# broadinstitute/delphy

Hardware: AMD Instinct MI355X
Metric: MCMC moves/sec on 100k-tip SARS-CoV-2 EMAT at 1/2/4/8 MI355X (higher is better)
Workload: dtype f64; 1 GPU; C4: synthetic 100000-tip EMAT, 29903 sites, HKY(kappa=5) + skygrid, 8092 partition parts (199999 nodes), 1000 moves/part/step, move mix 7.5/7.5/15/1/1; parts_per_gpu=8092, parts_requested=8192, max_part_nodes=-1, lds_staging=True, tickets_per_part_and_pass=4, parallelism=parts sharded over 1 GPU(s), one wavefront per part, collectives=none (one rank), emat_build_id=7d9b3896ecee7423

## Files before the change

### delphy_amd/csrc/emat_debug_host.hpp

```cpp
#ifndef EMAT_DEBUG_HOST_HPP_
#define EMAT_DEBUG_HOST_HPP_

namespace {

emat_status debug_settle(emat_backend* h, bool need_derived) {
  emat_status st = emat_synchronize(h); if (st) return st;
  st = sync_model_to_device(h); if (st) return st;
  st = materialize(h); if (st) return st;
  return need_derived && !h->derived_valid ? launch_recalc(h) : EMAT_OK;
}

}

extern "C" {

emat_status emat_debug_slab_layout(emat_backend* h, int32_t part_id, uint32_t* out8) {
  if (!h || !out8 || part_id < 0 || part_id >= (int)h->parts.size()) return EMAT_ERR_INVALID_ARGUMENT;
  if (!h->have_coal) return fail(h, EMAT_ERR_STATE, "no coalescent parts built");
  const PartHost& ph = h->parts[part_id];
  const int trace_cap = h->cfg.trace_moves > 0 ? h->cfg.trace_moves : 0;
  const uint32_t content = heap_content_bytes(ph.tree);
  const SlabGeo g = slab_geometry(h, ph.tree.num_nodes(), ph.tree.num_muts(), content, (int)ph.coal.k_bar_p.size(), ph.includes_run_root, ph.space_boost, ph.cell_boost);
  out8[0] = (uint32_t)sizeof(SlabHeader); out8[1] = (uint32_t)ph.tree.num_nodes() * (uint32_t)sizeof(NodeRec) + miss_dl_bytes_for((uint32_t)ph.tree.num_nodes()); out8[2] = a16((uint32_t)g.cell_cap * cell_bytes_for(ph.includes_run_root));
  out8[3] = a16((uint32_t)trace_cap * 32u); out8[4] = content; out8[5] = g.heap; out8[6] = g.scratch; out8[7] = (uint32_t)g.cell_cap;
  return EMAT_OK;
}
emat_status emat_debug_gamma(emat_backend* h, int32_t mode, int32_t n, const double* a, const double* x_or_q, double* out) {
  if (!h || n < 0 || (mode != 0 && mode != 1) || (n > 0 && (!a || !x_or_q || !out))) return EMAT_ERR_INVALID_ARGUMENT;
  if (h->host_only) return no_device(h);
  if (!bind_device(h)) return fail(h, EMAT_ERR_HIP, "hipSetDevice failed");
  if (n == 0) return EMAT_OK;
  DevBuf<double> da, dx, dout;
  HIP_TRY(da.upload(a, (size_t)n)); HIP_TRY(dx.upload(x_or_q, (size_t)n)); HIP_TRY(dout.upload(x_or_q, (size_t)n));
  hipLaunchKernelGGL(k_debug_gamma, dim3((unsigned)((n + 63) / 64)), dim3(64), 0, h->stream, da.p, dx.p, dout.p, n, mode);
  HIP_TRY(hipGetLastError());
  HIP_TRY(hipStreamSynchronize(h->stream));
  HIP_TRY(hipMemcpy(out, dout.p, (size_t)n * sizeof(double), hipMemcpyDeviceToHost));
  return EMAT_OK;
}
emat_status emat_debug_pop(emat_backend* h, const emat_pop_model* pm, int32_t op, int32_t n, const double* a, const double* b, double* out) {
  if (!h || !pm || n < 0 || op < 0 || op > 2 || (n > 0 && (!a || !b || !out))) return EMAT_ERR_INVALID_ARGUMENT;
  if (h->host_only) return no_device(h);
  if (!bind_device(h)) return fail(h, EMAT_ERR_HIP, "hipSetDevice failed");
  if (n == 0) return EMAT_OK;
  HostPopModel hp;
  try { hp = HostPopModel::from_c(*pm); } catch (const std::exception& ex) { return fail(h, EMAT_ERR_INVALID_ARGUMENT, ex.what()); }
  DevBuf<double> dx, dg, da, db, dout;
  HIP_TRY(dx.upload(hp.x.data(), hp.x.size())); HIP_TRY(dg.upload(hp.gamma.data(), hp.gamma.size()));
  HIP_TRY(da.upload(a, (size_t)n)); HIP_TRY(db.upload(b, (size_t)n)); HIP_TRY(dout.alloc((size_t)n));
  PopTable pt{};
  pt.kind = hp.kind; pt.skygrid_type = hp.skygrid_type; pt.skygrid_num_knots = (int)hp.x.size();
  for (int i = 0; i < 4; ++i) pt.p[i] = hp.p[i];
  pt.t_c = hp.t_c; pt.skygrid_x = dx.p; pt.skygrid_gamma = dg.p;
  pt.skygrid_inv_dx = (hp.x.size() >= 2 && hp.x.back() > hp.x.front()) ? (double)(hp.x.size() - 1) / (hp.x.back() - hp.x.front()) : 0.0;
  hipLaunchKernelGGL(k_debug_pop, dim3((unsigned)((n + 63) / 64)), dim3(64), 0, h->stream, pt, (int)op, da.p, db.p, dout.p, (int)n);
  HIP_TRY(hipGetLastError());
  HIP_TRY(hipStreamSynchronize(h->stream));
  HIP_TRY(hipMemcpy(out, dout.p, (size_t)n * sizeof(double), hipMemcpyDeviceToHost));
  return EMAT_OK;
}
emat_status emat_debug_interval_op(emat_backend* h, int32_t op, const int32_t* a, int32_t na, const int32_t* b, int32_t nb, int32_t* out, int32_t* n_out) {
  if (!h || !n_out || na < 0 || nb < 0 || (na > 0 && !a) || (nb > 0 && !b) || !out) return EMAT_ERR_INVALID_ARGUMENT;
  if (h->host_only) return no_device(h);
  if (!bind_device(h)) return fail(h, EMAT_ERR_HIP, "hipSetDevice failed");
  DevBuf<IvRec> dA, dB, dO; DevBuf<int> dn;
  HIP_TRY(dA.upload((const IvRec*)a, (size_t)na)); HIP_TRY(dB.upload((const IvRec*)b, (size_t)(op == 5 ? 0 : nb))); HIP_TRY(dO.alloc((size_t)(na + nb + 1))); HIP_TRY(dn.alloc(1));
  hipLaunchKernelGGL(k_debug_interval_op, dim3(1), dim3(64), 0, h->stream, (int)op, dA.p, (int)na, dB.p, (int)(op == 5 ? 0 : nb), op == 5 && nb > 0 ? b[0] : 0, dO.p, dn.p);
  HIP_TRY(hipGetLastError());
  HIP_TRY(hipStreamSynchronize(h->stream));
  int cnt = 0;
  HIP_TRY(hipMemcpy(&cnt, dn.p, sizeof(int), hipMemcpyDeviceToHost));
  if (cnt < 0) return fail(h, EMAT_ERR_INVALID_ARGUMENT, "emat_debug_interval_op: unknown op");
  *n_out = cnt;
  if (op <= 3 && cnt > 0) HIP_TRY(hipMemcpy(out, dO.p, (size_t)cnt * sizeof(IvRec), hipMemcpyDeviceToHost));
  return EMAT_OK;
}
emat_status emat_debug_tree_query(emat_backend* h, int32_t part_id, int32_t op, int32_t n, const int32_t* a, const int32_t* b, int32_t* out) {
  if (!h || n < 0 || (op != 0 && op != 1) || (n > 0 && (!a || !b || !out))) return EMAT_ERR_INVALID_ARGUMENT;
  if (h->host_only) return no_device(h);
  if (!bind_device(h)) return fail(h, EMAT_ERR_HIP, "hipSetDevice failed");
  if (part_id < 0 || part_id >= (int)h->parts.size()) return EMAT_ERR_INVALID_ARGUMENT;
  const int nn = h->parts[part_id].n_nodes;
  for (int i = 0; i < n; ++i) if (a[i] < -1 || a[i] >= nn || b[i] < -1 || b[i] >= nn) return fail(h, EMAT_ERR_INVALID_ARGUMENT, "emat_debug_tree_query: node index out of range");
  if (n == 0) return EMAT_OK;
  emat_status st = debug_settle(h, false); if (st) return st;
  DevBuf<int32_t> da, db, dout;
  HIP_TRY(da.upload(a, (size_t)n)); HIP_TRY(db.upload(b, (size_t)n)); HIP_TRY(dout.alloc((size_t)n));
  KernelArgs ka = make_args(h);
  hipLaunchKernelGGL(k_debug_tree_query, dim3(1), dim3(k_wave), 0, h->stream, ka, (int)part_id, (int)op, da.p, db.p, dout.p, (int)n);
  HIP_TRY(hipGetLastError());
  HIP_TRY(hipStreamSynchronize(h->stream));
  HIP_TRY(hipMemcpy(out, dout.p, (size_t)n * sizeof(int32_t), hipMemcpyDeviceToHost));
  return EMAT_OK;
}
emat_status emat_debug_miss_dl_check(emat_backend* h, int32_t* out_2n) {
  if (!h || !out_2n) return EMAT_ERR_INVALID_ARGUMENT;
  if (h->host_only) return no_device(h);
  if (!bind_device(h)) return fail(h, EMAT_ERR_HIP, "hipSetDevice failed");
  if (h->parts.empty()) return EMAT_OK;
  emat_status st = debug_settle(h, false); if (st) return st;
  DevBuf<int32_t> dout;
  HIP_TRY(dout.alloc(2 * h->parts.size()));
  return run_over_parts(h, k_debug_miss_dl_check, dout.p, out_2n, 2 * h->parts.size(), dout.p);
}
emat_status emat_debug_graft(emat_backend* h, int32_t part_id, int32_t X, double mu_proposal, int32_t mode, int32_t new_sibling, double new_t_P,
                             double* out, int32_t out_cap, int32_t* out_len) {
  if (!h || !out || !out_len || out_cap < 2 || mode < 0 || mode > 3) return EMAT_ERR_INVALID_ARGUMENT;
  if (h->host_only) return no_device(h);
  if (!bind_device(h)) return fail(h, EMAT_ERR_HIP, "hipSetDevice failed");
  if (part_id < 0 || part_id >= (int)h->parts.size()) return EMAT_ERR_INVALID_ARGUMENT;
  const int nn = h->parts[part_id].n_nodes;
  if (X < 0 || X >= nn || (mode == 3 && (new_sibling < 0 || new_sibling >= nn))) return fail(h, EMAT_ERR_INVALID_ARGUMENT, "emat_debug_graft: node index out of range");
  emat_status st = debug_settle(h, true); if (st) return st;
  DevBuf<double> dout; DevBuf<int32_t> dlen;
  HIP_TRY(dout.alloc((size_t)out_cap)); HIP_TRY(dlen.alloc(1));
  KernelArgs ka = make_args(h);
  hipLaunchKernelGGL(k_debug_graft, dim3(1), dim3(k_wave), 0, h->stream, ka, (int)part_id, (int)X, mu_proposal, (int)mode, (int)new_sibling, new_t_P, dout.p, (int)out_cap, dlen.p);
  HIP_TRY(hipGetLastError());
  HIP_TRY(hipStreamSynchronize(h->stream));
  HIP_TRY(hipMemcpy(out_len, dlen.p, sizeof(int32_t), hipMemcpyDeviceToHost));
  HIP_TRY(hipMemcpy(out, dout.p, (size_t)std::min(*out_len, out_cap) * sizeof(double), hipMemcpyDeviceToHost));
  if (mode >= 1) h->device_wrote_slabs();
  if (out[0] != 0.0) return fail(h, EMAT_ERR_INTERNAL, "emat_debug_graft: the device code stopped with part status " + std::to_string((int)out[0]));
  return *out_len > out_cap ? fail(h, EMAT_ERR_CAPACITY, "emat_debug_graft: out_cap too small") : EMAT_OK;
}
emat_status emat_debug_sample_history(emat_backend* h, int32_t part_id, int32_t n, const int32_t* branch, const double* t_end, const uint8_t* start_seq, double T, double mu,
                                      int32_t* counts, double* muts, int32_t muts_cap, int32_t* num_muts) {
// ... 134 lines not shown
```

### delphy_amd/csrc/emat_device_core.hpp

```cpp
#ifndef EMAT_DEV_NS
#error "define EMAT_DEV_NS and EMAT_VARIANT_LDS before including the device headers"
#endif

#include <hip/hip_runtime.h>
#include <cfloat>
#include <cstdint>

#include "emat_slab.hpp"

#ifndef EMAT_DEVICE_COMMON_ONCE_
#define EMAT_DEVICE_COMMON_ONCE_
namespace emat {
extern __shared__ __attribute__((aligned(16))) uint8_t emat_lds[];
constexpr uint32_t k_lds_tables_bytes = k_max_lds_partitions * (1 + 4 + 16) * 8;
constexpr uint32_t k_lds_ctx_bytes = 288;
#ifndef EMAT_RNG_BLOCKS
#define EMAT_RNG_BLOCKS 32
#endif
constexpr uint32_t k_rng_blocks = EMAT_RNG_BLOCKS;
static_assert(k_rng_blocks == 0 || (k_rng_blocks <= 64 && (k_rng_blocks & (k_rng_blocks - 1)) == 0), "one block per lane, a power of two");
constexpr uint32_t k_lds_rng_bytes = k_rng_blocks * 16;
constexpr uint32_t k_lds_static_bytes = k_lds_tables_bytes + k_lds_ctx_bytes + k_lds_rng_bytes + k_max_lds_partitions * 16 * 8;
__shared__ __attribute__((aligned(16))) uint8_t emat_lds_tables[k_lds_tables_bytes];
__shared__ __attribute__((aligned(16))) uint8_t emat_lds_ctx[k_lds_ctx_bytes];
// ... 366 lines not shown
  }
  if (inside) { dst[out].start = cs; dst[out].end = ce; ++out; }
  return out;
}
EMAT_D int iv_intersect(IvRec* dst, const IvRec* A, int nA, const IvRec* B, int nB) {
  int out = 0, ia = 0, ib = 0;
  while (ia != nA && ib != nB) {
    int so = A[ia].start > B[ib].start ? A[ia].start : B[ib].start;
    int eo = A[ia].end < B[ib].end ? A[ia].end : B[ib].end;
    if (so < eo) { dst[out].start = so; dst[out].end = eo; ++out; }
    if (A[ia].end <= B[ib].end) ++ia; else ++ib;
  }
  return out;
}
EMAT_D bool iv_intersects(const IvRec* A, int nA, const IvRec* B, int nB) {
  int ia = 0, ib = 0;
  while (ia != nA && ib != nB) {
    int so = A[ia].start > B[ib].start ? A[ia].start : B[ib].start;
    int eo = A[ia].end < B[ib].end ? A[ia].end : B[ib].end;
    if (so < eo) return true;
    if (A[ia].end <= B[ib].end) ++ia; else ++ib;
  }
  return false;
}
EMAT_D int iv_subtract(IvRec* dst, const IvRec* A, int nA, const IvRec* B, int nB) {
  if (nA == 0) return 0;
  int out = 0, ia = 0, ib = 0;
  int cs = A[0].start, ce = A[0].end;
  while (ia != nA) {
    bool next = false;
    if (ib == nB) { dst[out].start = cs; dst[out].end = ce; ++out; next = true; }
    else {
      int bs = B[ib].start, be = B[ib].end;
      if (bs < cs) {
        if (be <= cs) ++ib;
        else if (be < ce) { cs = be; ++ib; }
        else next = true;
      } else if (bs < ce) {
        if (cs < bs) { dst[out].start = cs; dst[out].end = bs; ++out; }
        if (be < ce) { cs = be; ++ib; }
        else next = true;
      } else { dst[out].start = cs; dst[out].end = ce; ++out; next = true; }
    }
    if (next) { ++ia; if (ia != nA) { cs = A[ia].start; ce = A[ia].end; } }
  }
  return out;
}
EMAT_D SVec<IvRec> iv_subtract_sc(Ctx& c, const IvRec* A, int nA, const IvRec* B, int nB) {
  SVec<IvRec> r = sc_vec<IvRec>(c, nA + nB + 1);
  if (!c.failed) r.n = iv_subtract(r.p, A, nA, B, nB);
  sc_trim(c, r);
  return r;
}
EMAT_D SVec<IvRec> iv_copy_sc(Ctx& c, const IvRec* A, int nA) {
  SVec<IvRec> r = sc_vec<IvRec>(c, nA);
  if (!c.failed) { for (int i = 0; i < nA; ++i) r.p[i] = A[i]; r.n = nA; }
  return r;
}

EMAT_D int fs_lower_bound(const FsRec* v, int n, int l) { int lo = 0, hi = n; while (lo < hi) { int mid = (lo + hi) >> 1; if (v[mid].site < l) lo = mid + 1; else hi = mid; } return lo; }
EMAT_D bool miss_contains(Ctx& c, int node, int l) { return iv_contains(miss_of(c, node), (int)nodes_of(c)[node].miss.cnt, l); }
EMAT_D int miss_get_from_state(Ctx& c, int node, int l) {
  const FsRec* v = mfs_of(c, node); int n = (int)nodes_of(c)[node].mfs.cnt;
  int k = fs_lower_bound(v, n, l);
  return (k < n && v[k].site == l) ? (int)v[k].state : (int)c.ref[l];
}
EMAT_DN void miss_set_from_state(Ctx& c, int node, int l, int from) {
  ListRef& r = nodes_of(c)[node].mfs;
  FsRec* v = mfs_of(c, node); int n = (int)r.cnt;
  int k = fs_lower_bound(v, n, l);
  bool present = (k < n && v[k].site == l);
  if (from != (int)c.ref[l]) {
    miss_dl_forget(c, node);
    if (present) { v[k].state = (uint8_t)from; return; }
    list_reserve<FsRec>(c, r, n + 1);
    if (c.failed) return;
    v = mfs_of(c, node);
    for (int i = n; i > k; --i) v[i] = v[i - 1];
    v[k].site = l; v[k].state = (uint8_t)from; v[k].pad[0] = v[k].pad[1] = v[k].pad[2] = 0;
    set_list_cnt(c, r, n + 1);
  } else if (present) {
    miss_dl_forget(c, node);
    for (int i = k; i + 1 < n; ++i) v[i] = v[i + 1];
    set_list_cnt(c, r, n - 1);
  }
}

struct SdRec { int32_t site; uint8_t from, to; uint16_t pad; };
EMAT_D int sd_lower_bound(const SdRec* v, int n, int l) { int lo = 0, hi = n; while (lo < hi) { int mid = (lo + hi) >> 1; if (v[mid].site < l) lo = mid + 1; else hi = mid; } return lo; }
EMAT_D bool sd_contains(const SVec<SdRec>& v, int l) { int k = sd_lower_bound(v.p, v.n, l); return k < v.n && v.p[k].site == l; }
EMAT_DF void sd_insert_at(Ctx& c, SVec<SdRec>& v, int k, int site, int from, int to) {
  if (v.n >= v.cap) { EMAT_FAIL(c, k_part_overflow); return; }
  for (int i = v.n; i > k; --i) v.p[i] = v.p[i - 1];
  v.p[k].site = site; v.p[k].from = (uint8_t)from; v.p[k].to = (uint8_t)to; v.p[k].pad = 0; v.n++;
}
EMAT_DF void sd_erase_at(SVec<SdRec>& v, int k) { for (int i = k; i + 1 < v.n; ++i) v.p[i] = v.p[i + 1]; v.n--; }
EMAT_DN SVec<SdRec> sd_push_front_v(Ctx& c, SVec<SdRec> v, int site, int from, int to) {
  int k = sd_lower_bound(v.p, v.n, site);
  if (k < v.n && v.p[k].site == site) {
    EMAT_CHECK(c, to == (int)v.p[k].from);
    v.p[k].from = (uint8_t)from;
    if (v.p[k].from == v.p[k].to) sd_erase_at(v, k);
  } else sd_insert_at(c, v, k, site, from, to);
  return v;
}
EMAT_DF void sd_push_front(Ctx& c, SVec<SdRec>& v, int site, int from, int to) { v = sd_push_front_v(c, v, site, from, to); }
// ... 452 lines not shown
```

### delphy_amd/csrc/emat_device_spr.hpp

```cpp

#include "emat_device_core.hpp"

namespace emat {
namespace EMAT_DEV_NS {

EMAT_DN SVec<FsRec> fsv_set_v(Ctx& c, SVec<FsRec> v, int l, int from) {
  int k = fs_lower_bound(v.p, v.n, l);
  bool present = (k < v.n && v.p[k].site == l);
  if (from != (int)c.ref[l]) {
    if (present) { v.p[k].state = (uint8_t)from; return v; }
    if (v.n >= v.cap) { EMAT_FAIL(c, k_part_overflow); return v; }
    for (int i = v.n; i > k; --i) v.p[i] = v.p[i - 1];
    v.p[k].site = l; v.p[k].state = (uint8_t)from; v.p[k].pad[0] = v.p[k].pad[1] = v.p[k].pad[2] = 0; v.n++;
  } else if (present) { for (int i = k; i + 1 < v.n; ++i) v.p[i] = v.p[i + 1]; v.n--; }
  return v;
}
EMAT_DF void fsv_set(Ctx& c, SVec<FsRec>& v, int l, int from) { v = fsv_set_v(c, v, l, from); }

EMAT_DN void set_root_muts_from_deltas(Ctx& c, int root, const SVec<SdRec> d) { EMAT_TIMED(1);
  ListRef& r = nodes_of(c)[root].muts;
  list_reserve<MutRec>(c, r, d.n);
  if (c.failed) return;
  MutRec* m = list_ptr<MutRec>(c, r);
  for (int i = 0; i < d.n; ++i) { EMAT_CHECK(c, c.ref[d.p[i].site] == d.p[i].from); m[i] = make_mut(d.p[i].from, d.p[i].site, d.p[i].to, k_neg_dbl_max); }
// ... 531 lines not shown
  const double t_mut_X = 0.5 * (t_P + t_X);
  list_reserve<MutRec>(c, nodes_of(c)[X].muts, SPX.hot_deltas.n);
  if (!c.failed) {
    MutRec* m = muts_of(c, X);
    for (int i = 0; i < SPX.hot_deltas.n; ++i) m[i] = make_mut(SPX.hot_deltas.p[i].from, SPX.hot_deltas.p[i].site, SPX.hot_deltas.p[i].to, t_mut_X);
    set_list_cnt(c, nodes_of(c)[X].muts, SPX.hot_deltas.n);
  }
  set_root_muts_from_deltas(c, P, r2r);
  nodes_of(c)[P].lambda = calc_lambda_at_node(c, P);
  sc_release(c, mark);
}
EMAT_DN void apply_rooty_graft(Ctx& c, const Graft& g) { EMAT_TIMED(1);
  if (c.failed) return;
  const int X = g.X, P = nodes_of(c)[X].parent, S = sibling_of(c, P, X);
  const double t_X = nodes_of(c)[X].t, t_P = nodes_of(c)[P].t, t_S = nodes_of(c)[S].t;
  const BranchInfo& PX = g.bi[k_PX]; const BranchInfo& PS = g.bi[k_PS]; const BranchInfo& SPX = g.bi[k_SPX];
  EMAT_CHECK(c, nmuts(c, S) == 0);
  ScMark mark = sc_mark(c);
  nodes_of(c)[X].muts.cnt = 0;
  SVec<SdRec> r2r = deltas_from_root_muts(c, P, PX.hot_muts.n + PS.hot_muts.n + SPX.hot_muts.n);
  nodes_of(c)[P].muts.cnt = 0;
  for (int i = PX.hot_muts.n - 1; i >= 0 && !c.failed; --i) {
    const MutRec& m = PX.hot_muts.p[i];
    list_push<MutRec>(c, nodes_of(c)[X].muts, m);
    sd_push_back(c, r2r, m.site, m.to, m.from);
    miss_set_from_state(c, S, m.site, m.from);
  }
  for (int i = PS.hot_muts.n - 1; i >= 0 && !c.failed; --i) {
    const MutRec& m = PS.hot_muts.p[i];
    list_push<MutRec>(c, nodes_of(c)[S].muts, m);
    sd_push_back(c, r2r, m.site, m.to, m.from);
    miss_set_from_state(c, X, m.site, m.from);
  }
  for (int i = 0; i < SPX.hot_muts.n && !c.failed; ++i) {
    const MutRec& m = SPX.hot_muts.p[i];
    if (m.t > t_P) list_push<MutRec>(c, nodes_of(c)[X].muts, m);
    else { list_push<MutRec>(c, nodes_of(c)[S].muts, make_mut(m.to, m.site, m.from, t_P + (t_P - m.t))); sd_push_back(c, r2r, m.site, m.from, m.to); }
  }
  sort_muts(muts_of(c, X), nmuts(c, X)); sort_muts(muts_of(c, S), nmuts(c, S));
  set_root_muts_from_deltas(c, P, r2r);
  clamp_mut_times(muts_of(c, X), nmuts(c, X), t_P, t_X); clamp_mut_times(muts_of(c, S), nmuts(c, S), t_P, t_S);
  nodes_of(c)[P].lambda = nodes_of(c)[X].lambda - delta_lambda_across_branch(c, X);
  sc_release(c, mark);
}

EMAT_DN void start_inner_graft_analysis(Ctx& c, int X, Graft& g) { EMAT_TIMED(1);
  g.X = X; g.rooty = false; g.delta_log_G = g.log_alpha_mut = 0.0; g.nbi = 0; g.bi = nullptr;
  const int P = nodes_of(c)[X].parent;
  EMAT_CHECK(c, X != hdr_of(c)->root && P != hdr_of(c)->root);
  if (c.failed) return;
  const int S = sibling_of(c, P, X);
  const double t_X = nodes_of(c)[X].t, t_P = nodes_of(c)[P].t;
  g.S = S; g.t_P = t_P;
  int depth = 0, path_muts = 0;
  { EMAT_TIMED(1);
  for (int cur = X; cur != k_no_node; cur = nodes_of(c)[cur].parent) { ++depth; if (c.includes_run_root || nodes_of(c)[cur].parent != k_no_node) path_muts += nmuts(c, cur); } }
  int bi_cap = depth + 2 < 4 ? depth + 2 : 4;
  EMAT_TIMED_BLOCK(1, setup_timer);
  g.bi = (BranchInfo*)sc_alloc(c, (uint32_t)bi_cap * (uint32_t)sizeof(BranchInfo));
  if (c.failed) return;
  auto bi_room = [&]() {
    if (g.nbi < bi_cap) return;
    if (bi_cap >= depth + 2) { EMAT_FAIL(c, k_part_overflow); return; }
    const int ncap = 2 * bi_cap < depth + 2 ? 2 * bi_cap : depth + 2;
    BranchInfo* nb = (BranchInfo*)sc_alloc(c, (uint32_t)ncap * (uint32_t)sizeof(BranchInfo));
    if (c.failed) return;
    for (int i = 0; i < g.nbi; ++i) nb[i] = g.bi[i];
    g.bi = nb; bi_cap = ncap;
  };
  {
    BranchInfo& PX = g.bi[g.nbi++]; bi_init(PX);
    PX.A = P; PX.B = X; PX.is_open = false; PX.T_to_X = t_X - t_P;
    PX.warm = sc_vec<IvRec>(c, 1); { IvRec all; all.start = 0; all.end = c.L; push(c, PX.warm, all); }
    PX.hot = iv_subtract_sc(c, PX.warm.p, PX.warm.n, miss_of(c, S), (int)nodes_of(c)[S].miss.cnt);
  }
  SVec<IvRec> sl_iv = iv_copy_sc(c, miss_of(c, S), (int)nodes_of(c)[S].miss.cnt);
  SVec<FsRec> sl_fs = sc_vec<FsRec>(c, (int)nodes_of(c)[S].mfs.cnt + path_muts + 1);
  { const FsRec* f = mfs_of(c, S); for (int i = 0; i < (int)nodes_of(c)[S].mfs.cnt; ++i) push(c, sl_fs, f[i]); }
  {
    BranchInfo& PX = g.bi[0];
    PX.pl_A = nodes_of(c)[X].lambda;
    const MutRec* m = muts_of(c, X);
    for (int i = nmuts(c, X) - 1; i >= 0; --i) PX.pl_A += dq(c, m[i].site, m[i].to, m[i].from);
  }
  EMAT_TIMED_END(setup_timer);
  double next_pl_B;
  { EMAT_TIMED(1);
  next_pl_B = -1 * delta_lambda_across_node_missations(c, S); }
  g.bi[0].pl_A -= next_pl_B;
  int cur = P, parent = nodes_of(c)[cur].parent, sibling = sibling_of(c, parent, cur);
  double partial_lambda = next_pl_B;
  { EMAT_TIMED(1);
  while (sl_iv.n != 0 && !c.failed) {
    bi_room(); if (c.failed) break;
    BranchInfo& bi = g.bi[g.nbi++]; bi_init(bi);
    bi.A = parent; bi.B = cur; bi.is_open = false; bi.T_to_X = t_X - nodes_of(c)[parent].t;
    bi.warm = sl_iv;
    const MutRec* mc = muts_of(c, cur);
    for (int i = nmuts(c, cur) - 1; i >= 0; --i) {
      if (iv_contains(sl_iv.p, sl_iv.n, mc[i].site)) { partial_lambda += dq(c, mc[i].site, mc[i].to, mc[i].from); fsv_set(c, sl_fs, mc[i].site, mc[i].from); }
    }
    bi.hot = iv_subtract_sc(c, bi.warm.p, bi.warm.n, miss_of(c, sibling), (int)nodes_of(c)[sibling].miss.cnt);
    SVec<IvRec> new_sl = iv_subtract_sc(c, bi.warm.p, bi.warm.n, bi.hot.p, bi.hot.n);
    sl_iv = new_sl;
    { int w = 0; for (int i = 0; i < sl_fs.n; ++i) if (iv_contains(sl_iv.p, sl_iv.n, sl_fs.p[i].site)) sl_fs.p[w++] = sl_fs.p[i]; sl_fs.n = w; }
    next_pl_B = -1 * delta_lambda_across_missations(c, sl_iv.p, sl_iv.n, sl_fs.p, sl_fs.n);
    bi.pl_A = partial_lambda - next_pl_B;
    partial_lambda = next_pl_B;
    c.bytes += 64 + 16 * nmuts(c, cur) + 24 * ((int)nodes_of(c)[sibling].miss.cnt + bi.warm.n);
    if (parent != hdr_of(c)->root) {
      cur = parent; parent = nodes_of(c)[cur].parent; sibling = sibling_of(c, parent, cur);
    } else {
      if (!c.includes_run_root) { bi.hot = bi.warm; bi.pl_A += partial_lambda; }
      else if (sl_iv.n != 0) {
        bi_room(); if (c.failed) break;
        BranchInfo& fo = g.bi[g.nbi++]; bi_init(fo);
        fo.A = k_no_node; fo.B = hdr_of(c)->root; fo.is_open = true; fo.T_to_X = t_X - nodes_of(c)[parent].t;
        fo.warm = sl_iv; fo.hot = sl_iv; fo.pl_A = partial_lambda;
      }
      sl_iv.n = 0; sl_fs.n = 0;
    }
  } }
  if (c.failed) return;
  { EMAT_TIMED(1);
  struct Owned { MutRec m; int owner; int pad; };
  SVec<Owned> tmp = sc_vec<Owned>(c, path_muts + 1);
  for (int i = 0; i < g.nbi; ++i) {
    BranchInfo& bi_i = g.bi[i];
    if (bi_i.B == hdr_of(c)->root) continue;
    const MutRec* mb = muts_of(c, bi_i.B);
    for (int k = nmuts(c, bi_i.B) - 1; k >= 0; --k) {
      if (iv_contains(bi_i.warm.p, bi_i.warm.n, mb[k].site)) {
        bool found = false;
        for (int j = i; j < g.nbi; ++j) if (iv_contains(g.bi[j].hot.p, g.bi[j].hot.n, mb[k].site)) { Owned o; o.m = mb[k]; o.owner = j; o.pad = 0; push(c, tmp, o); found = true; break; }
        EMAT_CHECK(c, found);
      }
    }
  }
  if (tmp.n == 0) {
    for (int j = 0; j < g.nbi; ++j) { BranchInfo& bi = g.bi[j]; bi.hot_muts.p = nullptr; bi.hot_muts.n = bi.hot_muts.cap = 0; bi.hot_deltas.p = nullptr; bi.hot_deltas.n = bi.hot_deltas.cap = 0; bi.pl_X = bi.pl_A; }
  } else
  for (int j = 0; j < g.nbi && !c.failed; ++j) {
    BranchInfo& bi = g.bi[j];
    int cnt = 0; for (int k = 0; k < tmp.n; ++k) if (tmp.p[k].owner == j) ++cnt;
    bi.hot_muts = sc_vec<MutRec>(c, cnt);
    bi.hot_deltas = sc_vec<SdRec>(c, cnt);
    for (int k = tmp.n - 1; k >= 0; --k) if (tmp.p[k].owner == j) push(c, bi.hot_muts, tmp.p[k].m);
    bi.pl_X = bi.pl_A;
    for (int k = 0; k < bi.hot_muts.n; ++k) {
      const MutRec& m = bi.hot_muts.p[k];
      if (!bi.is_open) sd_push_back(c, bi.hot_deltas, m.site, m.from, m.to);
      bi.pl_X += dq(c, m.site, m.from, m.to);
    }
  } }
  return;
}
EMAT_DF void propose_new_inner_graft_mutations(Ctx& c, Graft& g) { EMAT_TIMED(1);
  const int X = g.X;
  for (int idx = 0; idx < g.nbi && !c.failed; ++idx) {
    BranchInfo& bi = g.bi[idx];
    if (bi.hot.n == 0) { EMAT_CHECK(c, bi.hot_muts.n == 0); continue; }
    SVec<MutRec> nm = sample_history_for(c, bi);
    if (nm.n != 0) { EMAT_TIMED(1);
      filter_not_hot(nm, bi.hot);
      if (bi.B == X) {
        int w = 0;
        for (int i = 0; i < nm.n; ++i) {
          bool drop = !sd_contains(bi.hot_deltas, nm.p[i].site) && is_site_missing_at(c, X, nm.p[i].site);
          if (!drop) nm.p[w++] = nm.p[i];
        }
        nm.n = w;
      }
      adjust_mutational_history(c, nm, bi.hot_deltas, X, nodes_of(c)[X].t);
    }
    bi.hot_muts = nm;
    recompute_open_pl_A(c, bi);
  }
}
EMAT_DF void finish_inner_graft_analysis(Ctx& c, Graft& g) { EMAT_TIMED(1);
  if (c.failed || g.nbi == 0) return;
  const int X = g.X; const double t_X = nodes_of(c)[X].t;
  g.delta_log_G = 0.0;
  for (int i = 0; i < g.nbi; ++i) { BranchInfo& bi = g.bi[i]; g.delta_log_G += branch_log_G(c, t_X - bi.T_to_X, t_X, bi.pl_X, bi.hot_muts.p, bi.hot_muts.n); }
  BranchInfo& last = g.bi[g.nbi - 1];
  if (last.is_open) for (int i = 0; i < last.hot_muts.n; ++i) g.delta_log_G += log_pi_ratio(c, last.hot_muts.p[i]);
  g.log_alpha_mut = 0.0;
  for (int i = 0; i < g.nbi; ++i) {
    BranchInfo& bi = g.bi[i];
    int Ls = iv_num_sites(bi.hot.p, bi.hot.n);
    if (bi.B == X) Ls = (c.L - nodes_of(c)[X].n_missing) - (iv_num_sites(bi.warm.p, bi.warm.n) - iv_num_sites(bi.hot.p, bi.hot.n));
    g.log_alpha_mut += log_alpha_mut_term(c.mu_prop, Ls, bi.T_to_X, bi.hot_muts.n, bi.is_open, bi.hot_deltas.n);
  }
}
EMAT_D void recalc_lambda_along_hot_path(Ctx& c, const Graft& g) {
  for (int i = 0; i + 1 < g.nbi; ++i) { int A = g.bi[i].A, B = g.bi[i].B; nodes_of(c)[A].lambda = nodes_of(c)[B].lambda - delta_lambda_across_branch(c, B); }
}
EMAT_D void erase_marked_muts(Ctx& c, int node) { MutRec* m = muts_of(c, node); int n = nmuts(c, node), w = 0; for (int i = 0; i < n; ++i) if (m[i].site != -1) m[w++] = m[i]; set_list_cnt(c, nodes_of(c)[node].muts, w); }
EMAT_DF void peel_inner_graft(Ctx& c, const Graft& g) { EMAT_TIMED(1);
  if (c.failed || g.nbi == 0) return;
  const int X = g.X, P = nodes_of(c)[X].parent, root = hdr_of(c)->root;
  const double t_X = nodes_of(c)[X].t, t_P = nodes_of(c)[P].t;
  const BranchInfo& fin = g.bi[g.nbi - 1];
  ScMark mark = sc_mark(c);
  SVec<SdRec> r2r; r2r.p = nullptr; r2r.n = r2r.cap = 0;
  if (fin.is_open) r2r = deltas_from_root_muts(c, root, path_mut_count(c, X));
// ... 691 lines not shown
```

### delphy_amd/csrc/emat_part_kernels.hpp

```cpp
#ifndef EMAT_PART_KERNELS_HPP_
#define EMAT_PART_KERNELS_HPP_

#if defined(EMAT_PROFILE_PHASES) || defined(EMAT_COUNT_CALLS)
namespace emat {
constexpr int k_fn_replicas = 64;
__device__ unsigned long long g_fn_ticks[k_fn_replicas * 3 * 2048][2];
__device__ unsigned g_fn_min_list_bytes = 0;
__shared__ int s_fn_count_me;
struct FnTimer {
  int key; long long t0;
  __device__ FnTimer(int k) : key(k), t0(clock64()) {}
  __device__ void stop() { if (key >= 0) { this->~FnTimer(); key = -1; } }
  __device__ ~FnTimer() { if (key >= 0 && threadIdx.x == 0 && s_fn_count_me) { const long long dt = clock64() - t0; unsigned long long* e = g_fn_ticks[(blockIdx.x & (k_fn_replicas - 1)) * (3 * 2048) + key]; atomicAdd(&e[0], (unsigned long long)dt); atomicAdd(&e[1], 1ull); } }
};
}
#endif
#ifdef EMAT_PROFILE_PHASES
namespace emat { __device__ unsigned long long g_arena_site_bytes[2048][2]; }
#endif
#define EMAT_DEV_NS dev_lds
#define EMAT_VARIANT_LDS 1
#include "emat_device_moves.hpp"
#undef EMAT_DEV_NS
#undef EMAT_VARIANT_LDS
// ... 632 lines not shown
  dev::Ctx c;
  init_ctx(c, slab, slab, a, tables);
  const int n = c.H->n_nodes, root = c.H->root;
  const bool root_part = c.includes_run_root;
  double tmin = dev::k_inf, tmax = -dev::k_inf, acc = 0.0;
  for (int i = lane; i < n; i += k_wave) {
    const double t = c.N[i].t;
    tmin = tmin < t ? tmin : t; tmax = tmax > t ? tmax : t;
    if (!dev::is_tip(c, i)) acc -= log(dev::pop_at_time(*c.pop, t));
  }
  for (int off = 32; off > 0; off >>= 1) { double o = __shfl_down(tmin, off, k_wave); tmin = tmin < o ? tmin : o; o = __shfl_down(tmax, off, k_wave); tmax = tmax > o ? tmax : o; }
  tmin = __shfl(tmin, 0, k_wave); tmax = __shfl(tmax, 0, k_wave);
  acc = wave_sum(acc);
  auto cell_of = [&](double t) { return (int)floor((t - t_ref) / t_step); };
  const int jlo = cell_of(tmin);
  int jhi = cell_of(tmax); if (jhi > -1) jhi = -1;
  const int cnt = jhi >= jlo ? jhi - jlo + 1 : 0;
  double* row = out + out_off[part];
  const bool fits = (uint32_t)cnt <= out_cap[part];
  if (fits) {
    for (int j = jlo + lane; j <= jhi; j += k_wave) {
      const double ub_j = t_ref + (double)(j + 1) * t_step;
      double sum = 0.0;
      for (int i = 0; i < n; ++i) {
        const double t = c.N[i].t;
        const int cs = cell_of(t);
        if (j < cs) continue;
        double w = dev::is_tip(c, i) ? -1.0 : +1.0;
        if (i == root && !root_part) w += 1.0;
        sum += (j == cs) ? w * (ub_j - t) / t_step : w;
      }
      row[j - jlo] = sum;
    }
  }
  if (lane == 0) { double* m = meta + (size_t)part * 4; m[0] = (double)jlo; m[1] = (double)cnt; m[2] = acc; m[3] = fits ? 0.0 : 1.0; }
}

__global__ void __launch_bounds__(k_wave) EMAT_OCCUPANCY k_debug_gamma(const double* a, const double* x, double* out, int n, int mode) {
  const int i = blockIdx.x * blockDim.x + threadIdx.x;
  if (i < n) out[i] = mode == 0 ? dev::gamma_q(a[i], x[i]) : dev::gamma_q_inv(a[i], x[i]);
}

__global__ void __launch_bounds__(k_wave) EMAT_OCCUPANCY k_debug_pop(PopTable pt, int op, const double* a, const double* b, double* out, int n) {
  const int i = blockIdx.x * blockDim.x + threadIdx.x;
  if (i < n) out[i] = op == 0 ? dev::pop_at_time(pt, a[i]) : op == 1 ? dev::pop_integral(pt, a[i], b[i]) : dev::pop_intensity_integral(pt, a[i], b[i]);
}
__global__ void k_debug_interval_op(int op, const IvRec* A, int nA, const IvRec* B, int nB, int site, IvRec* out, int* n_out) {
  if (threadIdx.x != 0 || blockIdx.x != 0) return;
  if (op == 1) *n_out = dev::iv_merge(out, A, nA, B, nB);
  else if (op == 2) *n_out = dev::iv_intersect(out, A, nA, B, nB);
  else if (op == 3) *n_out = dev::iv_subtract(out, A, nA, B, nB);
  else if (op == 5) *n_out = dev::iv_contains(A, nA, site) ? 1 : 0;
  else if (op == 6) *n_out = dev::iv_intersects(A, nA, B, nB) ? 1 : 0;
  else *n_out = -1;
}

}

#endif
```

### delphy_amd/engine.py

```python
from __future__ import annotations

import ctypes as C
import os
import subprocess
from dataclasses import dataclass, field
from typing import Optional, Sequence

import numpy as np

_HERE = os.path.dirname(os.path.abspath(__file__))
_CSRC = os.path.join(_HERE, "csrc")
_LIB_NAME = "libemat_hip.so"


class EmatError(RuntimeError):
    pass


STATUS_NAMES = {
    0: "EMAT_OK", 1: "EMAT_ERR_INVALID_ARGUMENT", 2: "EMAT_ERR_NO_DEVICE", 3: "EMAT_ERR_HIP", 4: "EMAT_ERR_STATE",
    5: "EMAT_ERR_CAPACITY", 6: "EMAT_ERR_INTERNAL", 7: "EMAT_ERR_BUFFER_TOO_SMALL", 8: "EMAT_ERR_IO",
}


# ... 735 lines not shown

    def num_muts_l(self) -> np.ndarray:
        out = np.zeros(self.num_sites, np.int32)
        self._ck(self._lib.emat_get_num_muts_l(self._h, out.ctypes.data_as(C.POINTER(C.c_int32))), "emat_get_num_muts_l")
        return out

    def scalable_coalescent_log_prior(self, t_ref: float, t_step: float) -> float:
        v = C.c_double()
        self._ck(self._lib.emat_get_scalable_coalescent_log_prior(self._h, t_ref, t_step, C.byref(v)), "emat_get_scalable_coalescent_log_prior")
        return float(v.value)

    def part_tree_lengths(self, num_parts: int) -> np.ndarray:
        out = np.zeros(num_parts)
        self._ck(self._lib.emat_get_part_tree_lengths(self._h, out.ctypes.data_as(C.POINTER(C.c_double))), "emat_get_part_tree_lengths")
        return out

    def Ttwiddle_l_partial(self, ext_offset, ext_node, ext_length):
        off = np.ascontiguousarray(ext_offset, np.int32); node = np.ascontiguousarray(ext_node, np.int32); val = np.ascontiguousarray(ext_length, np.float64)
        if node.shape[0] == 0:
            node = np.zeros(1, np.int32); val = np.zeros(1)
        S = np.zeros(self.num_sites); Rv = np.zeros(self.num_sites); T = C.c_double(0.0); dp = C.POINTER(C.c_double); ip = C.POINTER(C.c_int32)
        self._ck(self._lib.emat_Ttwiddle_l_partial(self._h, off.ctypes.data_as(ip), node.ctypes.data_as(ip), val.ctypes.data_as(dp), S.ctypes.data_as(dp), Rv.ctypes.data_as(dp), C.byref(T)),
                 "emat_Ttwiddle_l_partial")
        return S, Rv, float(T.value)

    def Ttwiddle_l_finish(self, S, R, tree_length: float) -> np.ndarray:
        S = np.ascontiguousarray(S, np.float64); R = np.ascontiguousarray(R, np.float64); out = np.zeros(self.num_sites); dp = C.POINTER(C.c_double)
        self._ck(self._lib.emat_Ttwiddle_l_finish(self._h, S.ctypes.data_as(dp), R.ctypes.data_as(dp), tree_length, out.ctypes.data_as(dp)), "emat_Ttwiddle_l_finish")
        return out

    def scalable_coalescent_partial(self, t_ref: float, t_step: float, first_cell: int, num_cells: int):
        kb = np.zeros(max(num_cells, 1)); logs = C.c_double(); need = C.c_int32()
        self._ck(self._lib.emat_scalable_coalescent_partial(self._h, t_ref, t_step, first_cell, num_cells, kb.ctypes.data_as(C.POINTER(C.c_double)), C.byref(logs), C.byref(need)),
                 "emat_scalable_coalescent_partial")
        return kb[:num_cells], float(logs.value), int(need.value)

    def scalable_coalescent_log_prior_from_grid(self, t_ref: float, t_step: float, first_cell: int, k_bar_sum: np.ndarray, sum_neg_log_pop: float) -> float:
        kb = np.ascontiguousarray(k_bar_sum, np.float64); v = C.c_double()
        self._ck(self._lib.emat_scalable_coalescent_log_prior(self._h, t_ref, t_step, first_cell, kb.shape[0], kb.ctypes.data_as(C.POINTER(C.c_double)), sum_neg_log_pop, C.byref(v)),
                 "emat_scalable_coalescent_log_prior")
        return float(v.value)

    def debug_pop(self, pop: PopModel, op: int, a, b) -> np.ndarray:
        a = np.ascontiguousarray(a, np.float64); b = np.ascontiguousarray(b, np.float64); out = np.zeros_like(a)
        m = pop.c_struct(); dp = C.POINTER(C.c_double)
        self._ck(self._lib.emat_debug_pop(self._h, C.byref(m), op, a.shape[0], a.ctypes.data_as(dp), b.ctypes.data_as(dp), out.ctypes.data_as(dp)), "emat_debug_pop")
        return out

    def debug_interval_op(self, op: int, a, b):
        A = np.ascontiguousarray(np.asarray(a, np.int32).reshape(-1, 2)); Bv = np.ascontiguousarray(np.asarray(b, np.int32).reshape(-1))
        nb = Bv.shape[0] if op == 5 else Bv.shape[0] // 2
        out = np.zeros((A.shape[0] + nb + 1, 2), np.int32); n = C.c_int32(); ip = C.POINTER(C.c_int32)
        self._ck(self._lib.emat_debug_interval_op(self._h, op, A.ctypes.data_as(ip), A.shape[0], Bv.ctypes.data_as(ip), nb, out.ctypes.data_as(ip), C.byref(n)), "emat_debug_interval_op")
        return out[: n.value].tolist() if op <= 3 else bool(n.value)

    def debug_tree_query(self, part: int, op: int, a, b) -> np.ndarray:
        a = np.ascontiguousarray(a, np.int32); b = np.ascontiguousarray(b, np.int32); out = np.zeros_like(a); ip = C.POINTER(C.c_int32)
        self._ck(self._lib.emat_debug_tree_query(self._h, part, op, a.shape[0], a.ctypes.data_as(ip), b.ctypes.data_as(ip), out.ctypes.data_as(ip)), "emat_debug_tree_query")
        return out

    def debug_graft(self, part: int, X: int, mu_proposal: float, mode: int = 0, new_sibling: int = 0, new_t_P: float = 0.0) -> dict:
        out = np.zeros(4096); n = C.c_int32()
        self._ck(self._lib.emat_debug_graft(self._h, part, X, mu_proposal, mode, new_sibling, new_t_P, out.ctypes.data_as(C.POINTER(C.c_double)), out.shape[0], C.byref(n)), "emat_debug_graft")
        return decode_graft_output(out[: n.value], mode)

    def debug_edit(self, part: int, X: int, ops):
        kind = np.array([{"slide": 0, "hop_up": 1, "flip": 2, "hop_down": 3}[o[0]] for o in ops], np.int32)
        node = np.array([int(o[1]) if o[0] == "hop_down" else -1 for o in ops], np.int32)
        t = np.array([float(o[1]) if o[0] == "slide" else 0.0 for o in ops], np.float64)
        self._ck(self._lib.emat_debug_edit(self._h, part, X, kind.shape[0], _ptr(kind, C.c_int32), _ptr(node, C.c_int32), _ptr(t, C.c_double)), "emat_debug_edit")

    def debug_sample_history(self, part: int, branch, t_end, start_seq, T: float, mu: float):
        branch = np.ascontiguousarray(branch, np.int32); t_end = np.ascontiguousarray(t_end, np.float64); seq = np.ascontiguousarray(start_seq, np.uint8)
        n = branch.shape[0]; cap = 64 * n + 1024
        counts = np.zeros(max(n, 1), np.int32); muts = np.zeros((cap, 4)); tot = C.c_int32()
        self._ck(self._lib.emat_debug_sample_history(self._h, part, n, _ptr(branch, C.c_int32), _ptr(t_end, C.c_double), _ptr(seq, C.c_uint8), T, mu,
                                                     _ptr(counts, C.c_int32), _ptr(muts, C.c_double), cap, C.byref(tot)), "emat_debug_sample_history")
        out, k = [], 0
        for i in range(n):
            out.append([[int(m[1]), int(m[0]), int(m[2]), float(m[3])] for m in muts[k: k + counts[i]]]); k += int(counts[i])
        return out

    def debug_gamma(self, mode: int, a, x_or_q) -> np.ndarray:
        a = np.ascontiguousarray(a, np.float64); x = np.ascontiguousarray(x_or_q, np.float64); out = np.zeros_like(a)
        dp = C.POINTER(C.c_double)
        self._ck(self._lib.emat_debug_gamma(self._h, mode, a.shape[0], a.ctypes.data_as(dp), x.ctypes.data_as(dp), out.ctypes.data_as(dp)), "emat_debug_gamma")
        return out

    def part_download(self, part: int) -> FlatTree:
        n, nm, ni, nf = C.c_int32(), C.c_int32(), C.c_int32(), C.c_int32()
        self._ck(self._lib.emat_part_get_sizes(self._h, part, C.byref(n), C.byref(nm), C.byref(ni), C.byref(nf)), "emat_part_get_sizes")
        t = FlatTree.empty(n.value, nm.value, ni.value, nf.value)
        v = t.c_view()
        self._ck(self._lib.emat_part_download(self._h, part, C.byref(v)), "emat_part_download")
        t.root = v.root
        return t.trimmed()

    def part_derived(self, part: int, num_nodes: int):
        lam = np.zeros(num_nodes)
        nmiss = np.zeros(num_nodes, np.int32)
        g, a = C.c_double(), C.c_double()
        self._ck(self._lib.emat_part_get_derived(self._h, part, _ptr(lam, C.c_double), _ptr(nmiss, C.c_int32), C.byref(g), C.byref(a)), "emat_part_get_derived")
        return lam, nmiss, float(g.value), float(a.value)

    def part_state_frequencies(self, part: int) -> np.ndarray:
        n = C.c_int32(8)
        counts = np.zeros((8, 4), np.int32)
# ... 340 lines not shown
```

Before: 486.7 million moves/s.

## Fuse interval subtractions into single split pass and drop root-path pre-walk in graft setup

Adds an iv_split routine that produces both the difference (hot) and the intersection remainder (sibling-missing intervals) in one merge pass, replacing two iv_subtract calls per branch in the SPR graft path walk. It removes the upfront walk from X to the root that counted depth and path mutations, and grows the branch-info and from-state buffers on demand instead. The per-branch filtering of sl_fs now uses a linear merge against the sorted interval list instead of a binary search per entry. Hot-mutation bucketing now counts owners during the first scan, which removes a per-branch rescan of tmp. Buffer growth may allocate more scratch, and the overflow check tied to depth is gone.

```diff
diff --git a/delphy_amd/csrc/emat_debug_host.hpp b/delphy_amd/csrc/emat_debug_host.hpp
--- a/delphy_amd/csrc/emat_debug_host.hpp
+++ b/delphy_amd/csrc/emat_debug_host.hpp
@@ -64,7 +64,7 @@
   if (h->host_only) return no_device(h);
   if (!bind_device(h)) return fail(h, EMAT_ERR_HIP, "hipSetDevice failed");
   DevBuf<IvRec> dA, dB, dO; DevBuf<int> dn;
-  HIP_TRY(dA.upload((const IvRec*)a, (size_t)na)); HIP_TRY(dB.upload((const IvRec*)b, (size_t)(op == 5 ? 0 : nb))); HIP_TRY(dO.alloc((size_t)(na + nb + 1))); HIP_TRY(dn.alloc(1));
+  HIP_TRY(dA.upload((const IvRec*)a, (size_t)na)); HIP_TRY(dB.upload((const IvRec*)b, (size_t)(op == 5 ? 0 : nb))); HIP_TRY(dO.alloc(2 * (size_t)(na + nb + 1))); HIP_TRY(dn.alloc(1));
   hipLaunchKernelGGL(k_debug_interval_op, dim3(1), dim3(64), 0, h->stream, (int)op, dA.p, (int)na, dB.p, (int)(op == 5 ? 0 : nb), op == 5 && nb > 0 ? b[0] : 0, dO.p, dn.p);
   HIP_TRY(hipGetLastError());
   HIP_TRY(hipStreamSynchronize(h->stream));
@@ -72,7 +72,7 @@
   HIP_TRY(hipMemcpy(&cnt, dn.p, sizeof(int), hipMemcpyDeviceToHost));
   if (cnt < 0) return fail(h, EMAT_ERR_INVALID_ARGUMENT, "emat_debug_interval_op: unknown op");
   *n_out = cnt;
-  if (op <= 3 && cnt > 0) HIP_TRY(hipMemcpy(out, dO.p, (size_t)cnt * sizeof(IvRec), hipMemcpyDeviceToHost));
+  if ((op <= 3 || op == 7 || op == 8) && cnt > 0) HIP_TRY(hipMemcpy(out, dO.p, (size_t)cnt * sizeof(IvRec), hipMemcpyDeviceToHost));
   return EMAT_OK;
 }
 emat_status emat_debug_tree_query(emat_backend* h, int32_t part_id, int32_t op, int32_t n, const int32_t* a, const int32_t* b, int32_t* out) {
diff --git a/delphy_amd/csrc/emat_device_core.hpp b/delphy_amd/csrc/emat_device_core.hpp
--- a/delphy_amd/csrc/emat_device_core.hpp
+++ b/delphy_amd/csrc/emat_device_core.hpp
@@ -442,6 +442,44 @@
   sc_trim(c, r);
   return r;
 }
+EMAT_D void iv_split(IvRec* diff, int& ndiff, IvRec* rest, int& nrest, const IvRec* A, int nA, const IvRec* B, int nB) {
+  int od = 0, orr = 0, ia = 0, ib = 0;
+  if (nA != 0) {
+    int cs = A[0].start, ce = A[0].end, g = cs;
+    while (ia != nA) {
+      bool next = false; int ds = 0, de = 0;
+      if (ib == nB) { ds = cs; de = ce; next = true; }
+      else {
+        int bs = B[ib].start, be = B[ib].end;
+        if (bs < cs) {
+          if (be <= cs) ++ib;
+          else if (be < ce) { cs = be; ++ib; }
+          else next = true;
+        } else if (bs < ce) {
+          if (cs < bs) { ds = cs; de = bs; }
+          if (be < ce) { cs = be; ++ib; }
+          else next = true;
+        } else { ds = cs; de = ce; next = true; }
+      }
+      if (ds < de) {
+        if (g < ds) { rest[orr].start = g; rest[orr].end = ds; ++orr; }
+        diff[od].start = ds; diff[od].end = de; ++od; g = de;
+      }
+      if (next) {
+        if (g < ce) { rest[orr].start = g; rest[orr].end = ce; ++orr; }
+        ++ia; if (ia != nA) { cs = A[ia].start; ce = A[ia].end; g = cs; }
+      }
+    }
+  }
+  ndiff = od; nrest = orr;
+}
+EMAT_D void iv_split_sc(Ctx& c, SVec<IvRec>& diff, SVec<IvRec>& rest, const IvRec* A, int nA, const IvRec* B, int nB) {
+  diff = sc_vec<IvRec>(c, nA + nB + 1);
+  rest = sc_vec<IvRec>(c, nA + nB + 1);
+  if (!c.failed) iv_split(diff.p, diff.n, rest.p, rest.n, A, nA, B, nB);
+  sc_trim(c, rest);
+  diff.cap = diff.n;
+}
 EMAT_D SVec<IvRec> iv_copy_sc(Ctx& c, const IvRec* A, int nA) {
   SVec<IvRec> r = sc_vec<IvRec>(c, nA);
   if (!c.failed) { for (int i = 0; i < nA; ++i) r.p[i] = A[i]; r.n = nA; }
diff --git a/delphy_amd/csrc/emat_device_spr.hpp b/delphy_amd/csrc/emat_device_spr.hpp
--- a/delphy_amd/csrc/emat_device_spr.hpp
+++ b/delphy_amd/csrc/emat_device_spr.hpp
@@ -607,31 +607,37 @@
   const int S = sibling_of(c, P, X);
   const double t_X = nodes_of(c)[X].t, t_P = nodes_of(c)[P].t;
   g.S = S; g.t_P = t_P;
-  int depth = 0, path_muts = 0;
-  { EMAT_TIMED(1);
-  for (int cur = X; cur != k_no_node; cur = nodes_of(c)[cur].parent) { ++depth; if (c.includes_run_root || nodes_of(c)[cur].parent != k_no_node) path_muts += nmuts(c, cur); } }
-  int bi_cap = depth + 2 < 4 ? depth + 2 : 4;
+  int bi_cap = 4;
   EMAT_TIMED_BLOCK(1, setup_timer);
   g.bi = (BranchInfo*)sc_alloc(c, (uint32_t)bi_cap * (uint32_t)sizeof(BranchInfo));
   if (c.failed) return;
   auto bi_room = [&]() {
     if (g.nbi < bi_cap) return;
-    if (bi_cap >= depth + 2) { EMAT_FAIL(c, k_part_overflow); return; }
-    const int ncap = 2 * bi_cap < depth + 2 ? 2 * bi_cap : depth + 2;
+    const int ncap = 2 * bi_cap;
     BranchInfo* nb = (BranchInfo*)sc_alloc(c, (uint32_t)ncap * (uint32_t)sizeof(BranchInfo));
     if (c.failed) return;
     for (int i = 0; i < g.nbi; ++i) nb[i] = g.bi[i];
     g.bi = nb; bi_cap = ncap;
   };
+  SVec<IvRec> sl_iv;
   {
     BranchInfo& PX = g.bi[g.nbi++]; bi_init(PX);
     PX.A = P; PX.B = X; PX.is_open = false; PX.T_to_X = t_X - t_P;
     PX.warm = sc_vec<IvRec>(c, 1); { IvRec all; all.start = 0; all.end = c.L; push(c, PX.warm, all); }
-    PX.hot = iv_subtract_sc(c, PX.warm.p, PX.warm.n, miss_of(c, S), (int)nodes_of(c)[S].miss.cnt);
-  }
-  SVec<IvRec> sl_iv = iv_copy_sc(c, miss_of(c, S), (int)nodes_of(c)[S].miss.cnt);
-  SVec<FsRec> sl_fs = sc_vec<FsRec>(c, (int)nodes_of(c)[S].mfs.cnt + path_muts + 1);
-  { const FsRec* f = mfs_of(c, S); for (int i = 0; i < (int)nodes_of(c)[S].mfs.cnt; ++i) push(c, sl_fs, f[i]); }
+    iv_split_sc(c, PX.hot, sl_iv, PX.warm.p, PX.warm.n, miss_of(c, S), (int)nodes_of(c)[S].miss.cnt);
+  }
+  int path_muts = nmuts(c, X);
+  SVec<FsRec> sl_fs;
+  { const int nf = (int)nodes_of(c)[S].mfs.cnt;
+    sl_fs = sc_vec<FsRec>(c, nf + nmuts(c, P) + 1);
+    if (!c.failed) { const FsRec* f = mfs_of(c, S); for (int i = 0; i < nf; ++i) sl_fs.p[i] = f[i]; sl_fs.n = nf; } }
+  auto fs_room = [&](int more) {
+    if (sl_fs.n + more <= sl_fs.cap) return;
+    SVec<FsRec> nv = sc_vec<FsRec>(c, 2 * sl_fs.cap > sl_fs.n + more ? 2 * sl_fs.cap : sl_fs.n + more);
+    if (c.failed) return;
+    for (int i = 0; i < sl_fs.n; ++i) nv.p[i] = sl_fs.p[i];
+    nv.n = sl_fs.n; sl_fs = nv;
+  };
   {
     BranchInfo& PX = g.bi[0];
     PX.pl_A = nodes_of(c)[X].lambda;
@@ -639,6 +645,7 @@
     for (int i = nmuts(c, X) - 1; i >= 0; --i) PX.pl_A += dq(c, m[i].site, m[i].to, m[i].from);
   }
   EMAT_TIMED_END(setup_timer);
+  if (c.failed) return;
   double next_pl_B;
   { EMAT_TIMED(1);
   next_pl_B = -1 * delta_lambda_across_node_missations(c, S); }
@@ -651,18 +658,24 @@
     BranchInfo& bi = g.bi[g.nbi++]; bi_init(bi);
     bi.A = parent; bi.B = cur; bi.is_open = false; bi.T_to_X = t_X - nodes_of(c)[parent].t;
     bi.warm = sl_iv;
-    const MutRec* mc = muts_of(c, cur);
-    for (int i = nmuts(c, cur) - 1; i >= 0; --i) {
+    const MutRec* mc = muts_of(c, cur); const int nc = nmuts(c, cur);
+    path_muts += nc;
+    fs_room(nc); if (c.failed) break;
+    for (int i = nc - 1; i >= 0; --i) {
       if (iv_contains(sl_iv.p, sl_iv.n, mc[i].site)) { partial_lambda += dq(c, mc[i].site, mc[i].to, mc[i].from); fsv_set(c, sl_fs, mc[i].site, mc[i].from); }
     }
-    bi.hot = iv_subtract_sc(c, bi.warm.p, bi.warm.n, miss_of(c, sibling), (int)nodes_of(c)[sibling].miss.cnt);
-    SVec<IvRec> new_sl = iv_subtract_sc(c, bi.warm.p, bi.warm.n, bi.hot.p, bi.hot.n);
-    sl_iv = new_sl;
-    { int w = 0; for (int i = 0; i < sl_fs.n; ++i) if (iv_contains(sl_iv.p, sl_iv.n, sl_fs.p[i].site)) sl_fs.p[w++] = sl_fs.p[i]; sl_fs.n = w; }
+    iv_split_sc(c, bi.hot, sl_iv, bi.warm.p, bi.warm.n, miss_of(c, sibling), (int)nodes_of(c)[sibling].miss.cnt);
+    { int w = 0, k = 0;
+      for (int i = 0; i < sl_fs.n; ++i) {
+        const int l = sl_fs.p[i].site;
+        while (k < sl_iv.n && sl_iv.p[k].end <= l) ++k;
+        if (k < sl_iv.n && sl_iv.p[k].start <= l) sl_fs.p[w++] = sl_fs.p[i];
+      }
+      sl_fs.n = w; }
     next_pl_B = -1 * delta_lambda_across_missations(c, sl_iv.p, sl_iv.n, sl_fs.p, sl_fs.n);
     bi.pl_A = partial_lambda - next_pl_B;
     partial_lambda = next_pl_B;
-    c.bytes += 64 + 16 * nmuts(c, cur) + 24 * ((int)nodes_of(c)[sibling].miss.cnt + bi.warm.n);
+    c.bytes += 64 + 16 * nc + 24 * ((int)nodes_of(c)[sibling].miss.cnt + bi.warm.n);
     if (parent != hdr_of(c)->root) {
       cur = parent; parent = nodes_of(c)[cur].parent; sibling = sibling_of(c, parent, cur);
     } else {
@@ -687,25 +700,30 @@
     for (int k = nmuts(c, bi_i.B) - 1; k >= 0; --k) {
       if (iv_contains(bi_i.warm.p, bi_i.warm.n, mb[k].site)) {
         bool found = false;
-        for (int j = i; j < g.nbi; ++j) if (iv_contains(g.bi[j].hot.p, g.bi[j].hot.n, mb[k].site)) { Owned o; o.m = mb[k]; o.owner = j; o.pad = 0; push(c, tmp, o); found = true; break; }
+        for (int j = i; j < g.nbi; ++j) if (iv_contains(g.bi[j].hot.p, g.bi[j].hot.n, mb[k].site)) { Owned o; o.m = mb[k]; o.owner = j; o.pad = 0; push(c, tmp, o); ++g.bi[j].hot_muts.cap; found = true; break; }
         EMAT_CHECK(c, found);
       }
     }
   }
   if (tmp.n == 0) {
     for (int j = 0; j < g.nbi; ++j) { BranchInfo& bi = g.bi[j]; bi.hot_muts.p = nullptr; bi.hot_muts.n = bi.hot_muts.cap = 0; bi.hot_deltas.p = nullptr; bi.hot_deltas.n = bi.hot_deltas.cap = 0; bi.pl_X = bi.pl_A; }
-  } else
-  for (int j = 0; j < g.nbi && !c.failed; ++j) {
-    BranchInfo& bi = g.bi[j];
-    int cnt = 0; for (int k = 0; k < tmp.n; ++k) if (tmp.p[k].owner == j) ++cnt;
-    bi.hot_muts = sc_vec<MutRec>(c, cnt);
-    bi.hot_deltas = sc_vec<SdRec>(c, cnt);
-    for (int k = tmp.n - 1; k >= 0; --k) if (tmp.p[k].owner == j) push(c, bi.hot_muts, tmp.p[k].m);
-    bi.pl_X = bi.pl_A;
-    for (int k = 0; k < bi.hot_muts.n; ++k) {
-      const MutRec& m = bi.hot_muts.p[k];
-      if (!bi.is_open) sd_push_back(c, bi.hot_deltas, m.site, m.from, m.to);
-      bi.pl_X += dq(c, m.site, m.from, m.to);
+  } else if (!c.failed) {
+    for (int j = 0; j < g.nbi; ++j) {
+      BranchInfo& bi = g.bi[j];
+      const int cnt = bi.hot_muts.cap;
+      bi.hot_muts = sc_vec<MutRec>(c, cnt);
+      bi.hot_deltas = sc_vec<SdRec>(c, cnt);
+    }
+    if (c.failed) return;
+    for (int k = tmp.n - 1; k >= 0; --k) { SVec<MutRec>& v = g.bi[tmp.p[k].owner].hot_muts; v.p[v.n++] = tmp.p[k].m; }
+    for (int j = 0; j < g.nbi && !c.failed; ++j) {
+      BranchInfo& bi = g.bi[j];
+      bi.pl_X = bi.pl_A;
+      for (int k = 0; k < bi.hot_muts.n; ++k) {
+        const MutRec& m = bi.hot_muts.p[k];
+        if (!bi.is_open) sd_push_back(c, bi.hot_deltas, m.site, m.from, m.to);
+        bi.pl_X += dq(c, m.site, m.from, m.to);
+      }
     }
   } }
   return;
diff --git a/delphy_amd/csrc/emat_part_kernels.hpp b/delphy_amd/csrc/emat_part_kernels.hpp
--- a/delphy_amd/csrc/emat_part_kernels.hpp
+++ b/delphy_amd/csrc/emat_part_kernels.hpp
@@ -708,6 +708,12 @@
   else if (op == 3) *n_out = dev::iv_subtract(out, A, nA, B, nB);
   else if (op == 5) *n_out = dev::iv_contains(A, nA, site) ? 1 : 0;
   else if (op == 6) *n_out = dev::iv_intersects(A, nA, B, nB) ? 1 : 0;
+  else if (op == 7 || op == 8) {
+    IvRec* rest = out + nA + nB + 1; int nd = 0, nr = 0;
+    dev::iv_split(out, nd, rest, nr, A, nA, B, nB);
+    if (op == 8) for (int k = 0; k < nr; ++k) out[k] = rest[k];
+    *n_out = op == 7 ? nd : nr;
+  }
   else *n_out = -1;
 }
 
diff --git a/delphy_amd/engine.py b/delphy_amd/engine.py
--- a/delphy_amd/engine.py
+++ b/delphy_amd/engine.py
@@ -811,7 +811,7 @@
         nb = Bv.shape[0] if op == 5 else Bv.shape[0] // 2
         out = np.zeros((A.shape[0] + nb + 1, 2), np.int32); n = C.c_int32(); ip = C.POINTER(C.c_int32)
         self._ck(self._lib.emat_debug_interval_op(self._h, op, A.ctypes.data_as(ip), A.shape[0], Bv.ctypes.data_as(ip), nb, out.ctypes.data_as(ip), C.byref(n)), "emat_debug_interval_op")
-        return out[: n.value].tolist() if op <= 3 else bool(n.value)
+        return out[: n.value].tolist() if op <= 3 or op in (7, 8) else bool(n.value)
 
     def debug_tree_query(self, part: int, op: int, a, b) -> np.ndarray:
         a = np.ascontiguousarray(a, np.int32); b = np.ascontiguousarray(b, np.int32); out = np.zeros_like(a); ip = C.POINTER(C.c_int32)
```

Result: faster. 492.6 million moves/s (median of 6 runs) (+1.2%).
